# showlab/UniVTG

Hardware: NVIDIA H100
Metric: video-query pairs/sec (fwd+bwd) (higher is better)
Workload: dtype f16

## Files before the change

univtg_b200/csrc/backward.cu:

```cuda
#include <math.h>
#include <stdlib.h>

#include "backward.h"
#include "kernels.h"
#include "ptx.cuh"

namespace uv {

template <int EPT>
__global__ void __launch_bounds__(128) layernorm_bwd_kernel(const LnBwdArgs a) {
  pdl_prologue();
  const DropSpec drop = drop_resolve(a.drop);
  __shared__ float s_red[2][4];
  const int tid = threadIdx.x, warp = tid >> 5, lane = tid & 31;
  float acc_g[EPT], acc_b[EPT], acc_c[EPT];
#pragma unroll
  for (int i = 0; i < EPT; ++i) acc_g[i] = acc_b[i] = acc_c[i] = 0.f;
  const float inv_d = 1.0f / (float)a.d;

  for (int row = blockIdx.x; row < a.rows; row += gridDim.x) {
    const float mean = a.mean[row], rstd = a.rstd[row];
    const float* dout = a.dout + (size_t)row * a.ld_dout;
    const float* y = a.y + (size_t)row * a.ld_y;
    float xh[EPT], g[EPT];
// ... 101 lines not shown
    for (int i = 0; i < NV; ++i) {
      const int j = (tid + 128 * i) * 4;
      const bool in = j < a.d;
#define UV_LNB(c)                                          \
  xh[i].c = in ? (yv[i].c - mean) * rstd : 0.f;            \
  g[i].c = dj[i].c * gam[i].c;                             \
  acc_g[i].c += dj[i].c * xh[i].c;                         \
  acc_b[i].c += dj[i].c;                                   \
  s1 += g[i].c;                                            \
  s2 += g[i].c * xh[i].c;
      UV_LNB(x) UV_LNB(y) UV_LNB(z) UV_LNB(w)
#undef UV_LNB
    }
    s1 = warp_sum(s1);
    s2 = warp_sum(s2);
    __syncthreads();
    if (lane == 0) {
      s_red[0][warp] = s1;
      s_red[1][warp] = s2;
    }
    __syncthreads();
    const float c1 = (s_red[0][0] + s_red[0][1] + s_red[0][2] + s_red[0][3]) * inv_d;
    const float c2 = (s_red[1][0] + s_red[1][1] + s_red[1][2] + s_red[1][3]) * inv_d;
    float rs = 1.f;
    if (a.row_scale != nullptr) rs = a.row_scale[a.L > 0 ? row / a.L : 0];
#pragma unroll
    for (int i = 0; i < NV; ++i) {
      const int j = (tid + 128 * i) * 4;
      if (j < a.d) {
        float4 dy;
        dy.x = rstd * (g[i].x - c1 - xh[i].x * c2);
        dy.y = rstd * (g[i].y - c1 - xh[i].y * c2);
        dy.z = rstd * (g[i].z - c1 - xh[i].z * c2);
        dy.w = rstd * (g[i].w - c1 - xh[i].w * c2);
        if (a.relu_mask_y) {
          if (!(yv[i].x > 0.f)) dy.x = 0.f;
          if (!(yv[i].y > 0.f)) dy.y = 0.f;
          if (!(yv[i].z > 0.f)) dy.z = 0.f;
          if (!(yv[i].w > 0.f)) dy.w = 0.f;
        }
        if (a.dy32) *reinterpret_cast<float4*>(a.dy32 + (size_t)row * a.d + j) = dy;
        const float4 br = make_float4(dy.x * rs, dy.y * rs, dy.z * rs, dy.w * rs);
        acc_c[i].x += br.x, acc_c[i].y += br.y, acc_c[i].z += br.z, acc_c[i].w += br.w;
        if (a.dbr16)
          *reinterpret_cast<uint2*>(a.dbr16 + (size_t)row * a.ld16 + j) =
              make_uint2(cvt16x2(br.x, br.y, a.fmt16), cvt16x2(br.z, br.w, a.fmt16));
      }
    }
    if (a.dbr16)
      for (int j = a.d + tid; j < a.ld16; j += 128) a.dbr16[(size_t)row * a.ld16 + j] = 0;
  }
#pragma unroll
  for (int i = 0; i < NV; ++i) {
    const int j = (tid + 128 * i) * 4;
    if (j < a.d) {
      const float ps = a.pgrad_scale;
      if (a.dgamma) red_add_f32x4(a.dgamma + j, make_float4(acc_g[i].x * ps, acc_g[i].y * ps, acc_g[i].z * ps, acc_g[i].w * ps));
      if (a.dbeta) red_add_f32x4(a.dbeta + j, make_float4(acc_b[i].x * ps, acc_b[i].y * ps, acc_b[i].z * ps, acc_b[i].w * ps));
      if (a.colsum) red_add_f32x4(a.colsum + j, make_float4(acc_c[i].x * ps, acc_c[i].y * ps, acc_c[i].z * ps, acc_c[i].w * ps));
    }
  }
}

template <int NV>
__global__ void __launch_bounds__(256) layernorm_bwd_warp_kernel(const LnBwdArgs a) {
  pdl_prologue();
  const DropSpec drop = drop_resolve(a.drop);
  extern __shared__ float s_part[];
  const int tid = threadIdx.x, warp = tid >> 5, lane = tid & 31;
  constexpr int D = NV * 128;
  float4 acc_g[NV], acc_b[NV], acc_c[NV];
#pragma unroll
  for (int i = 0; i < NV; ++i) acc_g[i] = acc_b[i] = acc_c[i] = make_float4(0.f, 0.f, 0.f, 0.f);
  const float inv_d = 1.0f / (float)D;
  for (int row = blockIdx.x * 8 + warp; row < a.rows; row += gridDim.x * 8) {
    float4 g[NV], xh[NV];
#pragma unroll
    for (int i = 0; i < NV; ++i) {
      const int j = (i * 32 + lane) * 4;
      g[i] = __ldg(reinterpret_cast<const float4*>(a.dout + (size_t)row * a.ld_dout + j));
      xh[i] = __ldg(reinterpret_cast<const float4*>(a.y + (size_t)row * a.ld_y + j));
    }
    const float mean = a.mean[row], rstd = a.rstd[row];
    float rs = 1.f;
    if (a.row_scale != nullptr) rs = a.row_scale[a.L > 0 ? row / a.L : 0];
    float s1 = 0.f, s2 = 0.f;
    unsigned int relu = 0u;
#pragma unroll
    for (int i = 0; i < NV; ++i) {
      const int j = (i * 32 + lane) * 4;
      if (a.dout_mul) {
        const float4 m = __ldg(reinterpret_cast<const float4*>(a.dout_mul + (size_t)row * D + j));
        g[i].x *= m.x, g[i].y *= m.y, g[i].z *= m.z, g[i].w *= m.w;
      } else if (drop.on) {
        const float4 m = drop_mul4(drop, (unsigned int)row, (unsigned int)j);
        g[i].x *= m.x, g[i].y *= m.y, g[i].z *= m.z, g[i].w *= m.w;
      }
      const float4 gam = __ldg(reinterpret_cast<const float4*>(a.gamma + j));
#define UV_LNW(c, bit)                                  \
  if (xh[i].c > 0.f) relu |= 1u << (4 * i + bit);       \
  xh[i].c = (xh[i].c - mean) * rstd;                    \
  acc_g[i].c += g[i].c * xh[i].c;                       \
  acc_b[i].c += g[i].c;                                 \
  g[i].c *= gam.c;                                      \
  s1 += g[i].c;                                         \
  s2 += g[i].c * xh[i].c;
      UV_LNW(x, 0) UV_LNW(y, 1) UV_LNW(z, 2) UV_LNW(w, 3)
#undef UV_LNW
    }
    const float c1 = warp_sum(s1) * inv_d, c2 = warp_sum(s2) * inv_d;
#pragma unroll
    for (int i = 0; i < NV; ++i) {
      const int j = (i * 32 + lane) * 4;
      float4 dy;
      dy.x = rstd * (g[i].x - c1 - xh[i].x * c2);
      dy.y = rstd * (g[i].y - c1 - xh[i].y * c2);
      dy.z = rstd * (g[i].z - c1 - xh[i].z * c2);
      dy.w = rstd * (g[i].w - c1 - xh[i].w * c2);
      if (a.relu_mask_y) {
        if (!(relu & (1u << (4 * i + 0)))) dy.x = 0.f;
        if (!(relu & (1u << (4 * i + 1)))) dy.y = 0.f;
        if (!(relu & (1u << (4 * i + 2)))) dy.z = 0.f;
        if (!(relu & (1u << (4 * i + 3)))) dy.w = 0.f;
      }
      if (a.dy32) *reinterpret_cast<float4*>(a.dy32 + (size_t)row * D + j) = dy;
      const float4 br = make_float4(dy.x * rs, dy.y * rs, dy.z * rs, dy.w * rs);
      acc_c[i].x += br.x, acc_c[i].y += br.y, acc_c[i].z += br.z, acc_c[i].w += br.w;
      if (a.dbr16)
        *reinterpret_cast<uint2*>(a.dbr16 + (size_t)row * a.ld16 + j) = make_uint2(cvt16x2(br.x, br.y, a.fmt16), cvt16x2(br.z, br.w, a.fmt16));
    }
  }
  auto flush = [&](const float4 (&acc)[NV], float* dst) {
    if (dst == nullptr) return;
    __syncthreads();
#pragma unroll
    for (int i = 0; i < NV; ++i) *reinterpret_cast<float4*>(s_part + (size_t)warp * D + (i * 32 + lane) * 4) = acc[i];
    __syncthreads();
    for (int j = tid * 4; j < D; j += 256 * 4) {
      float4 t = make_float4(0.f, 0.f, 0.f, 0.f);
#pragma unroll
      for (int w = 0; w < 8; ++w) {
        const float4 v = *reinterpret_cast<const float4*>(s_part + (size_t)w * D + j);
        t.x += v.x, t.y += v.y, t.z += v.z, t.w += v.w;
      }
      const float ps = a.pgrad_scale;
      red_add_f32x4(dst + j, make_float4(t.x * ps, t.y * ps, t.z * ps, t.w * ps));
    }
  };
  flush(acc_g, a.dgamma);
  flush(acc_b, a.dbeta);
  flush(acc_c, a.colsum);
}

constexpr int kLnParamRows = 16;
__global__ void __launch_bounds__(256) layernorm_bwd_params_kernel(const LnBwdArgs a) {
  pdl_prologue();
  const DropSpec drop = drop_resolve(a.drop);
  const int jj = blockIdx.x * 256 + threadIdx.x;
  const bool in = jj < a.d;
  const int j = in ? jj : a.d - 1;
  const int r0 = blockIdx.y * kLnParamRows;
  const int r1 = min(a.rows, r0 + kLnParamRows);
  float ag = 0.f, ab = 0.f;
#pragma unroll
  for (int rr = 0; rr < kLnParamRows; ++rr) {
    const int r = r0 + rr;
    if (r >= r1) break;
    float dj = __ldg(a.dout + (size_t)r * a.ld_dout + j);
    if (a.dout_mul) dj *= __ldg(a.dout_mul + (size_t)r * a.d + j);
    else if (drop.on) {
      uint4 blk = make_uint4(0u, 0u, 0u, 0u);
      if ((threadIdx.x & 7) == 0) blk = drop_block(drop, (unsigned int)r, (unsigned int)(jj >> 3));
      const int src = (threadIdx.x & 31) & ~7;
      blk.x = __shfl_sync(0xffffffffu, blk.x, src);
      blk.y = __shfl_sync(0xffffffffu, blk.y, src);
      blk.z = __shfl_sync(0xffffffffu, blk.z, src);
      blk.w = __shfl_sync(0xffffffffu, blk.w, src);
      dj *= drop_pick(drop, blk, (unsigned int)(j & 7));
    }
    const float yv = a.y16 ? ld16(__ldg(a.y16 + (size_t)r * a.ld_y + j), a.y_fmt) : __ldg(a.y + (size_t)r * a.ld_y + j);
    const float xh = (yv - __ldg(a.mean + r)) * __ldg(a.rstd + r);
    ag += dj * xh;
    ab += dj;
  }
  if (in && a.dgamma) atomicAdd(a.dgamma + j, ag * a.pgrad_scale);
  if (in && a.dbeta) atomicAdd(a.dbeta + j, ab * a.pgrad_scale);
}

int launch_layernorm_bwd(const LnBwdArgs& a, cudaStream_t stream, int* kernel_used) {
  if (a.rows <= 0) return 0;
  if (a.dy32 == nullptr && a.dbr16 == nullptr) {
    if (kernel_used) *kernel_used = LNB_PARAMS;
    launch_k(layernorm_bwd_params_kernel, dim3(dim3((a.d + 255) / 256, (a.rows + kLnParamRows - 1) / kLnParamRows)), dim3(256), 0, stream, a);
    cudaError_t e = cudaGetLastError();
    if (e != cudaSuccess) set_error("layernorm_bwd launch failed: %s", cudaGetErrorString(e));
    return (int)e;
  }
  if (a.y16 != nullptr) {
    set_error("layernorm_bwd: a 16-bit LayerNorm input is only supported for the first projector layer (parameter gradients only)");
    return (int)cudaErrorInvalidValue;
  }
  static int max_blocks = 0;
  if (max_blocks == 0) {
    const char* e = getenv("UNIVTG_LNB_GRID");
    max_blocks = (e != nullptr && atoi(e) > 0) ? atoi(e) : 592;
  }
  const int grid = a.rows < max_blocks ? a.rows : max_blocks;
  const bool vec = a.d % 4 == 0 && a.ld_dout % 4 == 0 && a.ld_y % 4 == 0 && (!a.dbr16 || a.ld16 % 4 == 0) &&
                   (((uintptr_t)a.dout | (uintptr_t)a.y | (uintptr_t)a.gamma | (uintptr_t)a.dy32 | (uintptr_t)a.dout_mul) & 15) == 0 &&
                   (((uintptr_t)a.dgamma | (uintptr_t)a.dbeta | (uintptr_t)a.colsum) & 15) == 0 && ((uintptr_t)a.dbr16 & 7) == 0;
  static int use_warp = -1;
  if (use_warp < 0) {
    const char* e = getenv("UNIVTG_LNB_WARP");
    use_warp = (e != nullptr && e[0] == '0') ? 0 : 1;
  }
  const bool warp_ok = use_warp && vec && (a.d == 256 || a.d == 512 || a.d == 1024) && (!a.dbr16 || a.ld16 == a.d);
  if (warp_ok) {
    int dev = 0, sms = 132;
    cudaGetDevice(&dev);
    cudaDeviceGetAttribute(&sms, cudaDevAttrMultiProcessorCount, dev);
    int wgrid = (a.rows + 7) / 8;
    if (wgrid > sms) wgrid = sms;
    const size_t smem = (size_t)8 * a.d * sizeof(float);
    if (a.d == 1024) launch_k(layernorm_bwd_warp_kernel<8>, dim3(wgrid), dim3(256), smem, stream, a);
    else if (a.d == 512) launch_k(layernorm_bwd_warp_kernel<4>, dim3(wgrid), dim3(256), smem, stream, a);
    else launch_k(layernorm_bwd_warp_kernel<2>, dim3(wgrid), dim3(256), smem, stream, a);
    if (kernel_used) *kernel_used = a.d == 1024 ? LNB_WARP8 : (a.d == 512 ? LNB_WARP4 : LNB_WARP2);
  } else if (vec && a.d <= 512) {
    launch_k(layernorm_bwd_vec_kernel<1>, dim3(grid), dim3(128), 0, stream, a);
    if (kernel_used) *kernel_used = LNB_VEC1;
  } else if (vec && a.d <= 1024) {
    launch_k(layernorm_bwd_vec_kernel<2>, dim3(grid), dim3(128), 0, stream, a);
    if (kernel_used) *kernel_used = LNB_VEC2;
  } else if (a.d <= 128 * 8) {
    launch_k(layernorm_bwd_kernel<8>, dim3(grid), dim3(128), 0, stream, a);
    if (kernel_used) *kernel_used = LNB_ROW8;
  } else if (a.d <= 128 * 24) {
    launch_k(layernorm_bwd_kernel<24>, dim3(grid), dim3(128), 0, stream, a);
    if (kernel_used) *kernel_used = LNB_ROW24;
  } else {
    set_error("layernorm_bwd: d %d > 3072 not supported", a.d);
    return (int)cudaErrorInvalidValue;
  }
  cudaError_t e = cudaGetLastError();
  if (e != cudaSuccess) set_error("layernorm_bwd launch failed: %s", cudaGetErrorString(e));
  return (int)e;
}

__device__ __forceinline__ long long txt_row(const TxtRows& t, int r) {
  const int b = r / t.L, l = r - b * t.L;
  return l >= t.Lv ? (long long)b * (t.L - t.Lv) + (l - t.Lv) : -1;
}

template <bool TXT>
__global__ void __launch_bounds__(256) cvt16_colsum_kernel(const float* __restrict__ in32, int ld_in, uint16_t* __restrict__ out16,
                                                          int ld_out, int rows, int cols, int fmt, float* __restrict__ colsum, float cscale,
                                                          const TxtRows txt) {
  pdl_prologue();
  const int c = (blockIdx.x * 256 + threadIdx.x) * 4;
  if (c >= cols) return;
  const int r0 = blockIdx.y * 32;
  float4 s = make_float4(0.f, 0.f, 0.f, 0.f);
  for (int r = r0; r < min(rows, r0 + 32); ++r) {
    const float4 v = *reinterpret_cast<const float4*>(in32 + (size_t)r * ld_in + c);
    const uint2 h = make_uint2(cvt16x2(v.x, v.y, fmt), cvt16x2(v.z, v.w, fmt));
    *reinterpret_cast<uint2*>(out16 + (size_t)r * ld_out + c) = h;
    if constexpr (TXT) {
      const long long tr = txt_row(txt, r);
      if (tr >= 0 && c < txt.txt_cols) *reinterpret_cast<uint2*>(txt.txt16 + tr * txt.txt_cols + c) = h;
    }
    s.x += v.x;
    s.y += v.y;
    s.z += v.z;
    s.w += v.w;
  }
  if (colsum) {
    atomicAdd(colsum + c, s.x * cscale);
    atomicAdd(colsum + c + 1, s.y * cscale);
    atomicAdd(colsum + c + 2, s.z * cscale);
    atomicAdd(colsum + c + 3, s.w * cscale);
  }
}

__global__ void __launch_bounds__(256) tap_interleave_kernel(const float* __restrict__ src, float* __restrict__ dst, size_t nc) {
  pdl_prologue();
  for (size_t i = (size_t)blockIdx.x * 256 + threadIdx.x; i < nc; i += (size_t)gridDim.x * 256) {
    const float a = __ldg(src + i), b = __ldg(src + nc + i), c = __ldg(src + 2 * nc + i);
    float* o = dst + 3 * i;
    o[0] = a;
    o[1] = b;
    o[2] = c;
  }
}
int launch_tap_interleave(const float* src, float* dst, int N, int C, cudaStream_t stream) {
  const size_t nc = (size_t)N * C;
  size_t blocks = (nc + 255) / 256;
  if (blocks > 2368) blocks = 2368;
  launch_k(tap_interleave_kernel, dim3((unsigned)blocks), dim3(256), 0, stream, src, dst, nc);
  cudaError_t e = cudaGetLastError();
  if (e != cudaSuccess) set_error("tap_interleave launch failed: %s", cudaGetErrorString(e));
  return (int)e;
}

constexpr int kColsumRows = 16;
template <bool TXT>
__global__ void __launch_bounds__(128) colsum16_kernel(const uint16_t* __restrict__ in16, int ld, int rows, int cols, int fmt,
                                                      float* __restrict__ colsum, float scale, const TxtRows txt) {
  pdl_prologue();
  const int c = (blockIdx.x * 128 + threadIdx.x) * 8;
  if (c >= cols) return;
  const int r0 = blockIdx.y * kColsumRows;
  uint4 q[kColsumRows];
#pragma unroll
  for (int k = 0; k < kColsumRows; ++k)
    q[k] = (r0 + k < rows) ? __ldg(reinterpret_cast<const uint4*>(in16 + (size_t)(r0 + k) * ld + c)) : make_uint4(0u, 0u, 0u, 0u);
  if constexpr (TXT) {
    if (c < txt.txt_cols) {
#pragma unroll
      for (int k = 0; k < kColsumRows; ++k) {
        const long long tr = r0 + k < rows ? txt_row(txt, r0 + k) : -1;
        if (tr >= 0) *reinterpret_cast<uint4*>(txt.txt16 + tr * txt.txt_cols + c) = q[k];
      }
    }
  }
  float s[8] = {0.f, 0.f, 0.f, 0.f, 0.f, 0.f, 0.f, 0.f};
#pragma unroll
  for (int k = 0; k < kColsumRows; ++k) {
    const uint32_t w[4] = {q[k].x, q[k].y, q[k].z, q[k].w};
#pragma unroll
    for (int i = 0; i < 4; ++i) {
      s[2 * i] += ld16((uint16_t)(w[i] & 0xffff), fmt);
      s[2 * i + 1] += ld16((uint16_t)(w[i] >> 16), fmt);
    }
  }
  red_add_f32x4(colsum + c, make_float4(s[0] * scale, s[1] * scale, s[2] * scale, s[3] * scale));
  red_add_f32x4(colsum + c + 4, make_float4(s[4] * scale, s[5] * scale, s[6] * scale, s[7] * scale));
}

int launch_colsum16(const uint16_t* in16, int ld, int rows, int cols, int fmt, float* colsum, float scale, cudaStream_t stream,
                    TxtRows txt) {
  if (cols % 8 != 0 || ld % 8 != 0 || (reinterpret_cast<uintptr_t>(in16) & 15) != 0 || (reinterpret_cast<uintptr_t>(colsum) & 15) != 0 ||
      (txt.txt16 && (txt.txt_cols % 8 != 0 || (reinterpret_cast<uintptr_t>(txt.txt16) & 15) != 0))) {
    set_error("colsum16: columns / leading dimension must be multiples of 8 and the pointers 16-byte aligned");
    return (int)cudaErrorInvalidValue;
  }
  const dim3 grid((cols / 8 + 127) / 128, (rows + kColsumRows - 1) / kColsumRows);
// ... 34 lines not shown
      const int c0 = base + lane * 8;
      const bool in = c0 < d;
      const uint4 x = in ? __ldg(reinterpret_cast<const uint4*>(dO + (size_t)row * d + c0)) : make_uint4(0u, 0u, 0u, 0u);
      const uint4 y = in ? __ldg(reinterpret_cast<const uint4*>(O + (size_t)row * d + c0)) : make_uint4(0u, 0u, 0u, 0u);
      const uint32_t xw[4] = {x.x, x.y, x.z, x.w}, yw[4] = {y.x, y.y, y.z, y.w};
      float s = 0.f;
#pragma unroll
      for (int k = 0; k < 4; ++k)
        s += ld16((uint16_t)(xw[k] & 0xffff), fmt_do) * ld16((uint16_t)(yw[k] & 0xffff), fmt_o) +
             ld16((uint16_t)(xw[k] >> 16), fmt_do) * ld16((uint16_t)(yw[k] >> 16), fmt_o);
      for (int o = lph >> 1; o > 0; o >>= 1) s += __shfl_xor_sync(0xffffffffu, s, o);
      if (in && (lane & (lph - 1)) == 0) delta[((size_t)b * H + c0 / dh) * L + i] = s;
    }
    return;
  }
  for (int h = 0; h < H; ++h) {
    float s = 0.f;
    for (int c = lane; c < dh; c += 32) {
      const size_t idx = (size_t)row * d + h * dh + c;
      s += ld16(dO[idx], fmt_do) * ld16(O[idx], fmt_o);
    }
    s = warp_sum(s);
    if (lane == 0) delta[((size_t)b * H + h) * L + i] = s;
  }
}

int launch_attn_delta(const uint16_t* dO, int fmt_do, const uint16_t* O, int fmt_o, float* delta, int B, int L, int H, int dh,
                      cudaStream_t stream, int* vec_used) {
  const int rows = B * L;
  const int d = H * dh;
  const int vec = (dh % 8 == 0) && ((dh / 8) & (dh / 8 - 1)) == 0 && dh <= 256 && (d % 8 == 0) && (256 % dh == 0 || dh == 256) &&
                  ((reinterpret_cast<uintptr_t>(dO) | reinterpret_cast<uintptr_t>(O)) & 15) == 0;
  if (vec_used) *vec_used = vec;
  launch_k(attn_delta_kernel, dim3((rows * 32 + 255) / 256), dim3(256), 0, stream, dO, fmt_do, O, fmt_o, delta, B, L, H, dh, vec ? 1 : 0);
  cudaError_t e = cudaGetLastError();
  if (e != cudaSuccess) set_error("attn_delta launch failed: %s", cudaGetErrorString(e));
  return (int)e;
}

template <int DROP>
__global__ void __launch_bounds__(128) attention_bwd_simt_kernel(const AttnBwdArgs a) {
  pdl_prologue();
  const DropSpec drop = drop_resolve(a.drop);
  extern __shared__ float s_buf[];
  const int warp = threadIdx.x >> 5, lane = threadIdx.x & 31;
  const int gw = blockIdx.x * 4 + warp;
  if (gw >= a.B * a.H * a.L) return;
  const int i = gw % a.L;
  const int h = (gw / a.L) % a.H;
  const int b = gw / (a.L * a.H);
  float* p_s = s_buf + (size_t)warp * 2 * a.L;
  float* ds_s = p_s + a.L;
  const size_t ld = (size_t)3 * a.d;
  const uint16_t* qrow = a.qkv + ((size_t)b * a.L + i) * ld + h * a.dh;
  const uint16_t* dorow = a.dO + ((size_t)b * a.L + i) * a.d + h * a.dh;
  const float lse = a.lse[((size_t)b * a.H + h) * a.L + i];
  const float dlt = a.delta[((size_t)b * a.H + h) * a.L + i];
  for (int j = lane; j < a.L; j += 32) {
    float p = 0.f, ds = 0.f;
    if (a.key_mask[(size_t)b * a.L + j] != 0.f) {
      const uint16_t* krow = a.qkv + ((size_t)b * a.L + j) * ld + a.d + h * a.dh;
      const uint16_t* vrow = a.qkv + ((size_t)b * a.L + j) * ld + 2 * a.d + h * a.dh;
      float s = 0.f, dp = 0.f;
      for (int c = 0; c < a.dh; ++c) {
        s += ld16(qrow[c], a.fmt_act) * ld16(krow[c], a.fmt_act);
        dp += ld16(dorow[c], a.fmt_grad) * ld16(vrow[c], a.fmt_act);
      }
      p = expf(s * a.scale - lse);
      if constexpr (DROP != 0) {
        const float m = attn_drop_mul1(drop, (unsigned int)(b * a.H + h), (unsigned int)i, (unsigned int)j);
        ds = p * (m * dp - dlt) * a.scale;
        p *= m;
      } else {
        ds = p * (dp - dlt) * a.scale;
      }
    }
    p_s[j] = p;
    ds_s[j] = ds;
  }
  __syncwarp();
  for (int c = lane; c < a.dh; c += 32) {
    const float qc = ld16(qrow[c], a.fmt_act);
    const float doc = ld16(dorow[c], a.fmt_grad);
    float dq = 0.f;
    for (int j = 0; j < a.L; ++j) {
      const float ds = ds_s[j], p = p_s[j];
      if (p == 0.f && ds == 0.f) continue;
      const size_t kbase = ((size_t)b * a.L + j) * ld;
      dq += ds * ld16(a.qkv[kbase + a.d + h * a.dh + c], a.fmt_act);
      atomicAdd(a.dqkv32 + kbase + a.d + h * a.dh + c, ds * qc);
      atomicAdd(a.dqkv32 + kbase + 2 * a.d + h * a.dh + c, p * doc);
    }
    atomicAdd(a.dqkv32 + ((size_t)b * a.L + i) * ld + h * a.dh + c, dq);
  }
}

int launch_attention_bwd_simt(const AttnBwdArgs& a, cudaStream_t stream, int* kernel_used) {
  const int warps = a.B * a.H * a.L;
  const size_t smem = attention_bwd_simt_smem(a.L);
  auto kern = a.drop.on ? attention_bwd_simt_kernel<1> : attention_bwd_simt_kernel<0>;
  if (kernel_used) *kernel_used = 8 + (a.drop.on ? 1 : 0);
  if (smem > 48 * 1024) {
    cudaError_t e = cudaFuncSetAttribute(kern, cudaFuncAttributeMaxDynamicSharedMemorySize, (int)smem);
    if (e != cudaSuccess) {
      set_error("attention_bwd_simt smem %zu: %s", smem, cudaGetErrorString(e));
      return (int)e;
    }
  }
  launch_k(kern, dim3((warps + 3) / 4), dim3(128), smem, stream, a);
  cudaError_t e = cudaGetLastError();
  if (e != cudaSuccess) set_error("attention_bwd_simt launch failed: %s", cudaGetErrorString(e));
  return (int)e;
}

__global__ void __launch_bounds__(256) head_dz_kernel(const HeadFinalBwdArgs a) {
  pdl_prologue();
  const int idx = blockIdx.x * blockDim.x + threadIdx.x;
  const int rows = a.B * (a.Lv + 1) + 2;
  if (idx >= rows) return;
  float4 out = make_float4(0.f, 0.f, 0.f, 0.f);
  const int m = idx - 1;
  if (m >= 0 && m < a.B * (a.Lv + 1)) {
    const int b = m / (a.Lv + 1), l = m - b * (a.Lv + 1);
    if (l < a.Lv) {
      const size_t k = (size_t)b * a.Lv + l;
      const float pc = a.pred_logits[k];
      const float s0 = -a.pred_spans[2 * k];
      const float s1 = a.pred_spans[2 * k + 1];
      out.x = a.in_scale * a.g_logits[k] * pc * (1.f - pc);
      out.y = -a.in_scale * a.g_spans[2 * k] * s0 * (1.f - s0);
      out.z = a.in_scale * a.g_spans[2 * k + 1] * s1 * (1.f - s1);
    }
  }
  *reinterpret_cast<float4*>(a.dz + (size_t)idx * 4) = out;
}

__global__ void __launch_bounds__(256) head_dh_kernel(const HeadFinalBwdArgs a) {
  pdl_prologue();
  const int gw = (blockIdx.x * blockDim.x + threadIdx.x) >> 5;
  const int lane = threadIdx.x & 31;
  const int Mh = a.B * (a.Lv + 1);
  if (gw >= Mh) return;
  const size_t row = (size_t)gw + 1;
  const int l = gw % (a.Lv + 1);
  const bool sep = (l == a.Lv);
  float dzc[3], dz0[3], dz1[3];
#pragma unroll
  for (int t = 0; t < 3; ++t) {
    const float4 v = *reinterpret_cast<const float4*>(a.dz + (row + 1 - t) * 4);
    dzc[t] = v.x;
    dz0[t] = v.y;
    dz1[t] = v.z;
  }
  for (int c = lane * 2; c < a.d; c += 64) {
    float gc[2] = {0.f, 0.f}, gs[2] = {0.f, 0.f};
    if (!sep) {
#pragma unroll
      for (int t = 0; t < 3; ++t) {
#pragma unroll
        for (int e = 0; e < 2; ++e) {
          gc[e] += dzc[t] * a.w_cls[(size_t)t * a.d + c + e];
          gs[e] += dz0[t] * a.w_span[(size_t)t * a.d + c + e] + dz1[t] * a.w_span[(size_t)(3 + t) * a.d + c + e];
        }
      }
      const uint32_t hc = *reinterpret_cast<const uint32_t*>(a.h_cls + row * a.d + c);
      const uint32_t hs = *reinterpret_cast<const uint32_t*>(a.h_span + row * a.d + c);
      if (!pos16((uint16_t)(hc & 0xffff))) gc[0] = 0.f;
      if (!pos16((uint16_t)(hc >> 16))) gc[1] = 0.f;
      if (!pos16((uint16_t)(hs & 0xffff))) gs[0] = 0.f;
      if (!pos16((uint16_t)(hs >> 16))) gs[1] = 0.f;
    }
    *reinterpret_cast<uint32_t*>(a.dh_cls + row * a.d + c) = cvt16x2(gc[0], gc[1], a.fmt_grad);
    *reinterpret_cast<uint32_t*>(a.dh_span + row * a.d + c) = cvt16x2(gs[0], gs[1], a.fmt_grad);
  }
}

constexpr int kHeadDwRows = 32;
__device__ __forceinline__ void ld8(const uint16_t* p, int fmt, float (&v)[8]) {
  const uint4 q = *reinterpret_cast<const uint4*>(p);
  const uint32_t w[4] = {q.x, q.y, q.z, q.w};
#pragma unroll
  for (int i = 0; i < 4; ++i) {
    v[2 * i] = ld16((uint16_t)(w[i] & 0xffff), fmt);
    v[2 * i + 1] = ld16((uint16_t)(w[i] >> 16), fmt);
  }
}
__global__ void __launch_bounds__(128) head_dw_kernel(const HeadFinalBwdArgs a) {
  pdl_prologue();
  const int c = (blockIdx.x * 128 + threadIdx.x) * 8;
  const int Mh = a.B * (a.Lv + 1);
  const int m0 = blockIdx.y * kHeadDwRows;
  const int m1 = min(Mh, m0 + kHeadDwRows);
  if (c < a.d) {
    float wc[3][8], w0[3][8], w1[3][8], cs_c[8], cs_s[8];
#pragma unroll
    for (int j = 0; j < 8; ++j) {
      cs_c[j] = cs_s[j] = 0.f;
#pragma unroll
      for (int t = 0; t < 3; ++t) wc[t][j] = w0[t][j] = w1[t][j] = 0.f;
    }
    float pc[8], cc[8], nc[8], ps[8], cu[8], ns[8];
    ld8(a.h_cls + (size_t)m0 * a.d + c, a.fmt_act, pc);
    ld8(a.h_span + (size_t)m0 * a.d + c, a.fmt_act, ps);
    ld8(a.h_cls + (size_t)(m0 + 1) * a.d + c, a.fmt_act, cc);
    ld8(a.h_span + (size_t)(m0 + 1) * a.d + c, a.fmt_act, cu);
    for (int m = m0; m < m1; ++m) {
      const size_t row = (size_t)m + 1;
      ld8(a.h_cls + (row + 1) * a.d + c, a.fmt_act, nc);
      ld8(a.h_span + (row + 1) * a.d + c, a.fmt_act, ns);
      const float4 dz = *reinterpret_cast<const float4*>(a.dz + row * 4);
      if (a.cs_cls) {
        float gc[8], gs[8];
        ld8(a.dh_cls + row * a.d + c, a.fmt_grad, gc);
        ld8(a.dh_span + row * a.d + c, a.fmt_grad, gs);
#pragma unroll
        for (int j = 0; j < 8; ++j) {
          cs_c[j] += gc[j];
          cs_s[j] += gs[j];
        }
      }
      if (dz.x != 0.f || dz.y != 0.f || dz.z != 0.f) {
#pragma unroll
        for (int j = 0; j < 8; ++j) {
          wc[0][j] += dz.x * pc[j];
          wc[1][j] += dz.x * cc[j];
          wc[2][j] += dz.x * nc[j];
          w0[0][j] += dz.y * ps[j];
          w0[1][j] += dz.y * cu[j];
          w0[2][j] += dz.y * ns[j];
          w1[0][j] += dz.z * ps[j];
          w1[1][j] += dz.z * cu[j];
          w1[2][j] += dz.z * ns[j];
        }
      }
#pragma unroll
      for (int j = 0; j < 8; ++j) {
        pc[j] = cc[j];
        cc[j] = nc[j];
        ps[j] = cu[j];
        cu[j] = ns[j];
      }
    }
    const float gsc = a.pgrad_scale;
    float* dsts[3] = {a.gw_cls + (size_t)c * 3, a.gw_span + (size_t)c * 3, a.gw_span + ((size_t)a.d + c) * 3};
#pragma unroll
    for (int w = 0; w < 3; ++w) {
      float flat[24];
#pragma unroll
      for (int j = 0; j < 8; ++j)
#pragma unroll
        for (int t = 0; t < 3; ++t) flat[j * 3 + t] = (w == 0 ? wc[t][j] : (w == 1 ? w0[t][j] : w1[t][j])) * gsc;
#pragma unroll
      for (int q = 0; q < 6; ++q)
        red_add_f32x4(dsts[w] + 4 * q, make_float4(flat[4 * q], flat[4 * q + 1], flat[4 * q + 2], flat[4 * q + 3]));
    }
    if (a.cs_cls) {
      red_add_f32x4(a.cs_cls + c, make_float4(cs_c[0] * gsc, cs_c[1] * gsc, cs_c[2] * gsc, cs_c[3] * gsc));
      red_add_f32x4(a.cs_cls + c + 4, make_float4(cs_c[4] * gsc, cs_c[5] * gsc, cs_c[6] * gsc, cs_c[7] * gsc));
      red_add_f32x4(a.cs_span + c, make_float4(cs_s[0] * gsc, cs_s[1] * gsc, cs_s[2] * gsc, cs_s[3] * gsc));
      red_add_f32x4(a.cs_span + c + 4, make_float4(cs_s[4] * gsc, cs_s[5] * gsc, cs_s[6] * gsc, cs_s[7] * gsc));
    }
  }
  if (blockIdx.x == 0 && threadIdx.x == 0) {
    float bc = 0.f, b0 = 0.f, b1 = 0.f;
    for (int m = m0; m < m1; ++m) {
      const float4 dz = *reinterpret_cast<const float4*>(a.dz + ((size_t)m + 1) * 4);
      bc += dz.x;
      b0 += dz.y;
      b1 += dz.z;
    }
    atomicAdd(a.gb_cls, bc * a.pgrad_scale);
    atomicAdd(a.gb_span, b0 * a.pgrad_scale);
    atomicAdd(a.gb_span + 1, b1 * a.pgrad_scale);
  }
}

int launch_head_final_bwd(const HeadFinalBwdArgs& a, cudaStream_t stream) {
  const int Mh = a.B * (a.Lv + 1);
  launch_k(head_dz_kernel, dim3((Mh + 2 + 255) / 256), dim3(256), 0, stream, a);
  launch_k(head_dh_kernel, dim3((Mh * 32 + 255) / 256), dim3(256), 0, stream, a);
  launch_k(head_dw_kernel, dim3((a.d + 1023) / 1024, (Mh + kHeadDwRows - 1) / kHeadDwRows), dim3(128), 0, stream, a);
  cudaError_t e = cudaGetLastError();
  if (e != cudaSuccess) set_error("head_final_bwd launch failed: %s", cudaGetErrorString(e));
  return (int)e;
}

__global__ void __launch_bounds__(256) pool_bwd_kernel(const PoolBwdArgs a) {
  pdl_prologue();
  extern __shared__ float sm[];
  float* s_da = sm;
  __shared__ float s_dot;
  const int b = blockIdx.x;
  const int warp = threadIdx.x >> 5, lane = threadIdx.x & 31, nw = blockDim.x >> 5;
  const float* xt = a.x_txt + (size_t)b * a.Lt * a.d;
  const float* g = a.g_pooled + (size_t)b * a.d;
  const float* al = a.alpha + (size_t)b * a.Lt;
  for (int l = warp; l < a.Lt; l += nw) {
    float s = 0.f;
    for (int j = lane; j < a.d; j += 32) s += g[j] * xt[(size_t)l * a.d + j];
    s = warp_sum(s);
    if (lane == 0) s_da[l] = s;
  }
  __syncthreads();
  if (warp == 0) {
    float s = 0.f;
    for (int l = lane; l < a.Lt; l += 32) s += al[l] * s_da[l];
    s = warp_sum(s);
    if (lane == 0) s_dot = s;
  }
  __syncthreads();
  const float dot = s_dot;
  for (int l = threadIdx.x; l < a.Lt; l += blockDim.x) s_da[l] = al[l] * (s_da[l] - dot);
  __syncthreads();
  for (int j = threadIdx.x; j < a.d; j += blockDim.x) {
    const float gj = g[j], wj = a.w[j];
    float dw = 0.f;
    for (int l = 0; l < a.Lt; ++l) {
      const float dl = s_da[l];
      a.dx_txt[((size_t)b * a.Lt + l) * a.d + j] = (al[l] * gj + dl * wj) * a.out_scale;
      dw += dl * xt[(size_t)l * a.d + j];
    }
    atomicAdd(a.gw + j, dw);
  }
}

int launch_pool_bwd(const PoolBwdArgs& a, cudaStream_t stream) {
  launch_k(pool_bwd_kernel, dim3(a.B), dim3(256), (size_t)a.Lt * sizeof(float), stream, a);
  cudaError_t e = cudaGetLastError();
  if (e != cudaSuccess) set_error("pool_bwd launch failed: %s", cudaGetErrorString(e));
  return (int)e;
}

__global__ void __launch_bounds__(256) stream_gather_kernel(const float* __restrict__ dx, int L, int off, const float* __restrict__ extra,
                                                           float extra_scale, uint16_t* __restrict__ out16,
                                                           float* __restrict__ colsum, float cscale, int B, int Ls, int d, int fmt) {
  pdl_prologue();
  const int c = (blockIdx.x * 256 + threadIdx.x) * 4;
  if (c >= d) return;
  const int r0 = blockIdx.y * 32;
  const int rows = B * Ls;
  float4 s = make_float4(0.f, 0.f, 0.f, 0.f);
  for (int r = r0; r < min(rows, r0 + 32); ++r) {
    const int b = r / Ls, l = r - b * Ls;
    float4 v = *reinterpret_cast<const float4*>(dx + ((size_t)b * L + off + l) * d + c);
    if (extra) {
      const float4 e = *reinterpret_cast<const float4*>(extra + (size_t)r * d + c);
      v.x += e.x * extra_scale;
      v.y += e.y * extra_scale;
      v.z += e.z * extra_scale;
      v.w += e.w * extra_scale;
    }
    *reinterpret_cast<uint2*>(out16 + (size_t)r * d + c) = make_uint2(cvt16x2(v.x, v.y, fmt), cvt16x2(v.z, v.w, fmt));
    s.x += v.x;
    s.y += v.y;
    s.z += v.z;
    s.w += v.w;
  }
  if (colsum) {
    atomicAdd(colsum + c, s.x * cscale);
    atomicAdd(colsum + c + 1, s.y * cscale);
    atomicAdd(colsum + c + 2, s.z * cscale);
    atomicAdd(colsum + c + 3, s.w * cscale);
  }
}

int launch_stream_gather(const float* dx_stream, int L, int off, const float* extra, float extra_scale, uint16_t* out16,
                         float* colsum, float colsum_scale, int B, int Ls, int d, int fmt, cudaStream_t stream) {
  dim3 grid((d / 4 + 255) / 256, (B * Ls + 31) / 32);
  launch_k(stream_gather_kernel, dim3(grid), dim3(256), 0, stream, dx_stream, L, off, extra, extra_scale, out16, colsum, colsum_scale, B, Ls, d, fmt);
  cudaError_t e = cudaGetLastError();
  if (e != cudaSuccess) set_error("stream_gather launch failed: %s", cudaGetErrorString(e));
  return (int)e;
}


template <int EPT>
__global__ void __launch_bounds__(128) txt_pos_bwd_kernel(const TxtPosBwdArgs a) {
  pdl_prologue();
  const DropSpec drop = drop_resolve(a.drop);
  __shared__ float s_red[2][2][4];
  const int l = blockIdx.x;
  const int tid = threadIdx.x, warp = tid >> 5, lane = tid & 31;
  const float* P = a.table + (size_t)l * a.d;
  float acc_p[EPT], acc_g[EPT], acc_b[EPT], pv[EPT], gam[EPT];
#pragma unroll
  for (int i = 0; i < EPT; ++i) {
    const int j = tid + 128 * i;
    acc_p[i] = acc_g[i] = acc_b[i] = 0.f;
    pv[i] = j < a.d ? P[j] : 0.f;
    gam[i] = j < a.d ? a.gamma[j] : 0.f;
  }
  for (int b = 0; b < a.B; ++b) {
    const size_t r = (size_t)b * a.Lt + l;
    const float mean = a.mean[r], rstd = a.rstd[r];
    float g[EPT], xh[EPT];
    float s1 = 0.f, s2 = 0.f;
#pragma unroll
    for (int i = 0; i < EPT; ++i) {
      const int j = tid + 128 * i;
      g[i] = xh[i] = 0.f;
      if (j < a.d) {
        float go = a.dpos[r * a.d + j];
        if (a.mul32) go *= a.mul32[r * a.d + j];
        else if (drop.on) go *= drop_mul1(drop, (unsigned int)r, (unsigned int)j);
        xh[i] = (a.xt[r * a.d + j] + pv[i] - mean) * rstd;
        acc_g[i] += go * xh[i];
        acc_b[i] += go;
        g[i] = go * gam[i];
        s1 += g[i];
        s2 += g[i] * xh[i];
      }
    }
    s1 = warp_sum(s1);
    s2 = warp_sum(s2);
    if (lane == 0) {
      s_red[b & 1][0][warp] = s1;
      s_red[b & 1][1][warp] = s2;
    }
    __syncthreads();
    const float m1 = (s_red[b & 1][0][0] + s_red[b & 1][0][1] + s_red[b & 1][0][2] + s_red[b & 1][0][3]) / (float)a.d;
    const float m2 = (s_red[b & 1][1][0] + s_red[b & 1][1][1] + s_red[b & 1][1][2] + s_red[b & 1][1][3]) / (float)a.d;
    float* dxr = a.dx + ((size_t)b * a.L + a.Lv + l) * a.d;
#pragma unroll
    for (int i = 0; i < EPT; ++i) {
      const int j = tid + 128 * i;
      if (j < a.d) {
        const float du = rstd * (g[i] - m1 - xh[i] * m2);
        acc_p[i] += du;
        dxr[j] += du;
      }
    }
  }
#pragma unroll
  for (int i = 0; i < EPT; ++i) {
    const int j = tid + 128 * i;
    if (j < a.d) {
      a.dtable[(size_t)l * a.d + j] = acc_p[i] * a.pgrad_scale;
      atomicAdd(a.dgamma + j, acc_g[i] * a.pgrad_scale);
      atomicAdd(a.dbeta + j, acc_b[i] * a.pgrad_scale);
    }
  }
}

int launch_txt_pos_bwd(const TxtPosBwdArgs& a, cudaStream_t stream) {
  if (a.d > 128 * 8) {
    set_error("txt_pos_bwd: hidden_dim %d > 1024 not supported", a.d);
    return (int)cudaErrorInvalidValue;
  }
  launch_k(txt_pos_bwd_kernel<8>, dim3(a.Lt), dim3(128), 0, stream, a);
  cudaError_t e = cudaGetLastError();
  if (e != cudaSuccess) set_error("txt_pos_bwd launch failed: %s", cudaGetErrorString(e));
  return (int)e;
}

}
```

univtg_b200/csrc/loss.cu:

```cuda
#include <math.h>

#include "kernels.h"
#include "loss.h"
#include "ptx.cuh"

namespace uv {

__global__ void __launch_bounds__(256) loss_cos_kernel(const LossArgs a) {
  pdl_prologue();
  const int gw = (blockIdx.x * blockDim.x + threadIdx.x) >> 5;
  const int lane = threadIdx.x & 31;
  const int n_in = a.B * a.Lv;
  if (gw >= n_in + a.B * a.B) return;
  int bv, lv, bt;
  if (gw < n_in) {
    bv = gw / a.Lv;
    lv = gw - bv * a.Lv;
    bt = bv;
  } else {
    const int k = gw - n_in;
    bv = k / a.B;
    bt = k - bv * a.B;
    lv = (int)a.pos_idx[bv];
  }
// ... 212 lines not shown
  v = warp_max(v);
  __syncthreads();
  if ((threadIdx.x & 31) == 0) s_red[threadIdx.x >> 5] = v;
  __syncthreads();
  float t = -INFINITY;
  const int nw = blockDim.x >> 5;
  for (int i = 0; i < nw; ++i) t = fmaxf(t, s_red[i]);
  return t;
}

__global__ void __launch_bounds__(1024) qfvs_loss_kernel(const QfvsLossArgs a) {
  pdl_prologue();
  __shared__ float s_red[32];
  __shared__ int s_cnt[32];
  const int tid = threadIdx.x, nt = blockDim.x, lane = tid & 31, warp = tid >> 5, nw = nt >> 5;
  const int n = a.B * a.Lv;
  const float inv_tau = 1.0f / a.temperature;
  int ranked = 0;
  float c_t = 0.f, c_pos = 0.f, c_bce = 0.f, c_zpos = 0.f, mx = -INFINITY, se = 0.f;
  for (int base = 0; base < n; base += nt) {
    const int i = base + tid;
    const bool keep = i < n && a.mask_gt[i] != 0;
    const unsigned bal = __ballot_sync(0xffffffffu, keep);
    if (lane == 0) s_cnt[warp] = __popc(bal);
    __syncthreads();
    int before = 0, total = 0;
    for (int w = 0; w < nw; ++w) {
      const int c = s_cnt[w];
      before += w < warp ? c : 0;
      total += c;
    }
    __syncthreads();
    if (i < n) {
      float t = 0.f;
      if (keep) {
        t = a.sal[ranked + before + __popc(bal & ((1u << lane) - 1u))];
        const float p = a.pred_logits[i];
        const float lp = fmaxf(logf(p), -100.f), l1p = fmaxf(logf(1.f - p), -100.f);
        c_t += t;
        c_bce += -(t * lp + (1.f - t) * l1p);
        const float z = (a.cos_in[i] + logf(a.vmask[i] + 1e-45f)) * inv_tau;
        if (t > 0.f) {
          c_pos += 1.f;
          c_zpos += z;
        }
        if (z > mx) {
          se = se * expf(mx - z) + 1.f;
          mx = z;
        } else {
          se += expf(z - mx);
        }
      }
      a.g_logits_f[i] = t;
      a.g_cos_in[i] = keep ? 1.f : 0.f;
    }
    ranked += total;
  }
  const float sum_t = block_sum(c_t, s_red);
  const float n_pos = block_sum(c_pos, s_red);
  const float bce = block_sum(c_bce, s_red);
  const float zpos = block_sum(c_zpos, s_red);
  const float zmax = block_max(mx, s_red);
  const float lse = zmax + logf(block_sum(mx == -INFINITY ? 0.f : se * expf(mx - zmax), s_red));
  const bool on = sum_t != 0.f;
  const bool sal_on = on && a.has_pos != 0;
  for (int i = tid; i < n; i += nt) {
    const float t = a.g_logits_f[i];
    const bool keep = a.g_cos_in[i] != 0.f;
    float gf = 0.f, gc = 0.f;
    if (keep && on) {
      const float p = a.pred_logits[i];
      gf = (p - t) / fmaxf(p * (1.f - p), 1e-12f) / sum_t;
    }
    if (keep && sal_on) {
      const float z = (a.cos_in[i] + logf(a.vmask[i] + 1e-45f)) * inv_tau;
      gc = (expf(z - lse) - (t > 0.f ? 1.f / n_pos : 0.f)) * inv_tau;
    }
    a.g_logits_f[i] = gf;
    a.g_cos_in[i] = gc;
    a.g_spans_b[2 * i] = 0.f;
    a.g_spans_b[2 * i + 1] = 0.f;
    a.g_spans_g[2 * i] = 0.f;
    a.g_spans_g[2 * i + 1] = 0.f;
  }
  if (tid == 0) {
    a.losses[0] = 0.f;
    a.losses[1] = 0.f;
    a.losses[2] = on ? bce / sum_t : 0.f;
    a.losses[3] = 0.f;
    a.losses[4] = sal_on ? lse - zpos / n_pos : 0.f;
  }
}

int launch_qfvs_loss_forward(const QfvsLossArgs& q, cudaStream_t stream) {
  LossArgs c = {};
  c.xv = q.xv;
  c.xt = q.xt;
  c.B = q.B;
  c.Lv = q.Lv;
  c.d = q.d;
  c.cos_in = q.cos_in;
  c.vnorm = q.vnorm;
  c.tnorm = q.tnorm;
  launch_k(loss_cos_kernel, dim3(q.B * q.Lv), dim3(32), 0, stream, c);
  launch_k(qfvs_loss_kernel, dim3(1), dim3(1024), 0, stream, q);
  cudaError_t e = cudaGetLastError();
  if (e != cudaSuccess) set_error("qfvs loss forward launch failed: %s", cudaGetErrorString(e));
  return (int)e;
}

__global__ void __launch_bounds__(256) loss_bwd_small_kernel(const LossBwdArgs a) {
  pdl_prologue();
  const int i = blockIdx.x * blockDim.x + threadIdx.x;
  const int n = a.B * a.Lv;
  if (i >= n) return;
  const float wb = a.w[0], wg = a.w[1], wf = a.w[2];
  a.d_logits[i] = wf * a.g_logits_f[i];
  a.d_spans[2 * i] = wb * a.g_spans_b[2 * i] + wg * a.g_spans_g[2 * i];
  a.d_spans[2 * i + 1] = wb * a.g_spans_b[2 * i + 1] + wg * a.g_spans_g[2 * i + 1];
}

__global__ void __launch_bounds__(256) loss_bwd_vid_kernel(const LossBwdArgs a) {
  pdl_prologue();
  const int gw = (blockIdx.x * blockDim.x + threadIdx.x) >> 5;
  const int lane = threadIdx.x & 31;
  if (gw >= a.B * a.Lv) return;
  const int b = gw / a.Lv, l = gw - b * a.Lv;
  const float w_inter = a.w[3], w_intra = a.w[4];
  const float un = a.vnorm[gw];
  const float gi = w_intra * a.g_cos_in[gw];
  const float ci = a.cos_in[gw];
  const bool is_pos = a.pos_idx != nullptr && (int)a.pos_idx[b] == l;
  const float* u = a.xv + (size_t)gw * a.d;
  float* out = a.d_xv + (size_t)gw * a.d;
  extern __shared__ float s_c1[];
  float* c1w = s_c1 + (size_t)(threadIdx.x >> 5) * a.B;
  const float s1 = gi / (un * a.tnorm[b]);
  float s2 = gi * ci / (un * un);
  if (is_pos) {
    float s2p = 0.f;
    for (int k = lane; k < a.B; k += 32) {
      const float gx = w_inter * a.g_sim[b * a.B + k];
      c1w[k] = gx / (un * a.tnorm[k]);
      s2p += gx * a.sim[b * a.B + k] / (un * un);
    }
    s2 += warp_sum(s2p);
    __syncwarp();
  }
  for (int j = lane * 4; j < a.d; j += 128) {
    const float4 x = *reinterpret_cast<const float4*>(u + j);
    const float4 t = *reinterpret_cast<const float4*>(a.xt + (size_t)b * a.d + j);
    float4 o = make_float4(s1 * t.x, s1 * t.y, s1 * t.z, s1 * t.w);
    if (is_pos) {
#pragma unroll 4
      for (int k = 0; k < a.B; ++k) {
        const float4 tk = *reinterpret_cast<const float4*>(a.xt + (size_t)k * a.d + j);
        const float c1 = c1w[k];
        o.x += c1 * tk.x;
        o.y += c1 * tk.y;
        o.z += c1 * tk.z;
        o.w += c1 * tk.w;
      }
    }
    o.x -= s2 * x.x;
    o.y -= s2 * x.y;
    o.z -= s2 * x.z;
    o.w -= s2 * x.w;
    *reinterpret_cast<float4*>(out + j) = o;
  }
}

__global__ void __launch_bounds__(128) loss_bwd_txt_kernel(const LossBwdArgs a) {
  pdl_prologue();
  extern __shared__ float s_coef[];
  int* s_row = reinterpret_cast<int*>(s_coef + a.Lv + a.B);
  __shared__ float s_red[4];
  const int b = blockIdx.x, tid = threadIdx.x;
  const float w_inter = a.w[3], w_intra = a.w[4];
  const float tn = a.tnorm[b];
  float part = 0.f;
  for (int l = tid; l < a.Lv; l += 128) {
    const int i = b * a.Lv + l;
    const float g = w_intra * a.g_cos_in[i];
    s_coef[l] = g / (a.vnorm[i] * tn);
    part += g * a.cos_in[i];
  }
  const int nk = a.pos_idx != nullptr ? a.B : 0;
  for (int k = tid; k < nk; k += 128) {
    const float g = w_inter * a.g_sim[k * a.B + b];
    const int i = k * a.Lv + (int)a.pos_idx[k];
    s_coef[a.Lv + k] = g / (a.vnorm[i] * tn);
    s_row[k] = i;
    part += g * a.sim[k * a.B + b];
  }
  part = warp_sum(part);
  if ((tid & 31) == 0) s_red[tid >> 5] = part;
  __syncthreads();
  const float c2 = (s_red[0] + s_red[1] + s_red[2] + s_red[3]) / (tn * tn);
  for (int j = blockIdx.y * 128 + tid; j < a.d; j += gridDim.y * 128) {
    float o = -c2 * a.xt[(size_t)b * a.d + j];
    const float* xv = a.xv + (size_t)b * a.Lv * a.d + j;
#pragma unroll 8
    for (int l = 0; l < a.Lv; ++l) o += s_coef[l] * xv[(size_t)l * a.d];
#pragma unroll 4
    for (int k = 0; k < nk; ++k) o += s_coef[a.Lv + k] * a.xv[(size_t)s_row[k] * a.d + j];
    a.d_xt[(size_t)b * a.d + j] = o;
  }
}

int launch_loss_backward(const LossBwdArgs& a, cudaStream_t stream) {
  const int n = a.B * a.Lv;
  launch_k(loss_bwd_small_kernel, dim3((n + 255) / 256), dim3(256), 0, stream, a);
  if (a.pos_idx == nullptr) {
    cudaMemsetAsync(a.d_xv, 0, (size_t)n * a.d * sizeof(float), stream);
    cudaMemsetAsync(a.d_xt, 0, (size_t)a.B * a.d * sizeof(float), stream);
    cudaError_t e0 = cudaGetLastError();
    if (e0 != cudaSuccess) set_error("loss backward launch failed: %s", cudaGetErrorString(e0));
    return (int)e0;
  }
  launch_k(loss_bwd_vid_kernel, dim3((n * 32 + 255) / 256), dim3(256), (size_t)8 * a.B * sizeof(float), stream, a);
  launch_k(loss_bwd_txt_kernel, dim3(a.B, (a.d + 127) / 128), dim3(128), (size_t)(a.Lv + 2 * a.B) * sizeof(float), stream, a);
  cudaError_t e = cudaGetLastError();
  if (e != cudaSuccess) set_error("loss backward launch failed: %s", cudaGetErrorString(e));
  return (int)e;
}

int launch_qfvs_loss_backward(const LossBwdArgs& a, cudaStream_t stream) {
  const int n = a.B * a.Lv;
  launch_k(loss_bwd_small_kernel, dim3((n + 255) / 256), dim3(256), 0, stream, a);
  launch_k(loss_bwd_vid_kernel, dim3((n * 32 + 255) / 256), dim3(256), (size_t)8 * a.B * sizeof(float), stream, a);
  launch_k(loss_bwd_txt_kernel, dim3(a.B, (a.d + 127) / 128), dim3(128), (size_t)(a.Lv + 2 * a.B) * sizeof(float), stream, a);
  cudaError_t e = cudaGetLastError();
  if (e != cudaSuccess) set_error("qfvs loss backward launch failed: %s", cudaGetErrorString(e));
  return (int)e;
}

}
```

Before: 6818.

## Restructure LN param-grad, stream gather and pool backward kernels for more parallelism and ILP

The LayerNorm parameter-gradient kernel now has each thread handle 8 columns with vectorized loads. It batches rows for memory-level parallelism, reduces across warps in shared memory, and picks rows-per-slice so the grid fills the SMs. The stream gather kernel also reduces in shared memory before issuing atomics and preloads several rows per thread. Pool backward is split across a second grid dimension over columns, and two loops get higher unroll pragmas. The aim is fewer global atomics and more parallelism in small backward kernels, at the cost of more registers and shared memory.

```diff
diff --git a/univtg_b200/csrc/backward.cu b/univtg_b200/csrc/backward.cu
--- a/univtg_b200/csrc/backward.cu
+++ b/univtg_b200/csrc/backward.cu
@@ -277,46 +277,91 @@
   flush(acc_c, a.colsum);
 }
 
-constexpr int kLnParamRows = 16;
-__global__ void __launch_bounds__(256) layernorm_bwd_params_kernel(const LnBwdArgs a) {
+constexpr int kLnParamBatch = 4;
+__global__ void __launch_bounds__(256) layernorm_bwd_params_kernel(const LnBwdArgs a, int rows_per_slice) {
   pdl_prologue();
   const DropSpec drop = drop_resolve(a.drop);
-  const int jj = blockIdx.x * 256 + threadIdx.x;
-  const bool in = jj < a.d;
-  const int j = in ? jj : a.d - 1;
-  const int r0 = blockIdx.y * kLnParamRows;
-  const int r1 = min(a.rows, r0 + kLnParamRows);
-  float ag = 0.f, ab = 0.f;
-#pragma unroll
-  for (int rr = 0; rr < kLnParamRows; ++rr) {
-    const int r = r0 + rr;
-    if (r >= r1) break;
-    float dj = __ldg(a.dout + (size_t)r * a.ld_dout + j);
-    if (a.dout_mul) dj *= __ldg(a.dout_mul + (size_t)r * a.d + j);
-    else if (drop.on) {
-      uint4 blk = make_uint4(0u, 0u, 0u, 0u);
-      if ((threadIdx.x & 7) == 0) blk = drop_block(drop, (unsigned int)r, (unsigned int)(jj >> 3));
-      const int src = (threadIdx.x & 31) & ~7;
-      blk.x = __shfl_sync(0xffffffffu, blk.x, src);
-      blk.y = __shfl_sync(0xffffffffu, blk.y, src);
-      blk.z = __shfl_sync(0xffffffffu, blk.z, src);
-      blk.w = __shfl_sync(0xffffffffu, blk.w, src);
-      dj *= drop_pick(drop, blk, (unsigned int)(j & 7));
-    }
-    const float yv = a.y16 ? ld16(__ldg(a.y16 + (size_t)r * a.ld_y + j), a.y_fmt) : __ldg(a.y + (size_t)r * a.ld_y + j);
-    const float xh = (yv - __ldg(a.mean + r)) * __ldg(a.rstd + r);
-    ag += dj * xh;
-    ab += dj;
-  }
-  if (in && a.dgamma) atomicAdd(a.dgamma + j, ag * a.pgrad_scale);
-  if (in && a.dbeta) atomicAdd(a.dbeta + j, ab * a.pgrad_scale);
+  __shared__ float s_acc[2][8][256];
+  const int tx = threadIdx.x & 31, ty = threadIdx.x >> 5;
+  const int j0 = (blockIdx.x * 32 + tx) * 8;
+  const int nc = max(0, min(8, a.d - j0));
+  const bool dvec = nc == 8 && (a.ld_dout & 3) == 0 && ((uintptr_t)a.dout & 15) == 0 && !a.dout_mul;
+  const bool yvec = nc == 8 && !a.y16 && (a.ld_y & 1) == 0 && ((uintptr_t)a.y & 7) == 0;
+  const int r0 = (blockIdx.y * 8 + ty) * rows_per_slice;
+  const int r1 = nc > 0 ? min(a.rows, r0 + rows_per_slice) : r0;
+  float ag[8], ab[8];
+#pragma unroll
+  for (int k = 0; k < 8; ++k) ag[k] = ab[k] = 0.f;
+  for (int rb = r0; rb < r1; rb += kLnParamBatch) {
+    float g[kLnParamBatch][8], y[kLnParamBatch][8];
+#pragma unroll
+    for (int q = 0; q < kLnParamBatch; ++q) {
+      const int r = min(rb + q, r1 - 1);
+      const float* dr = a.dout + (size_t)r * a.ld_dout + j0;
+      if (dvec) {
+        const float4 u = __ldg(reinterpret_cast<const float4*>(dr)), v = __ldg(reinterpret_cast<const float4*>(dr + 4));
+        g[q][0] = u.x, g[q][1] = u.y, g[q][2] = u.z, g[q][3] = u.w, g[q][4] = v.x, g[q][5] = v.y, g[q][6] = v.z, g[q][7] = v.w;
+      } else {
+#pragma unroll
+        for (int k = 0; k < 8; ++k) g[q][k] = k < nc ? __ldg(dr + k) * (a.dout_mul ? __ldg(a.dout_mul + (size_t)r * a.d + j0 + k) : 1.f) : 0.f;
+      }
+      if (yvec) {
+        const float* yr = a.y + (size_t)r * a.ld_y + j0;
+#pragma unroll
+        for (int k = 0; k < 4; ++k) {
+          const float2 t = __ldg(reinterpret_cast<const float2*>(yr + 2 * k));
+          y[q][2 * k] = t.x, y[q][2 * k + 1] = t.y;
+        }
+      } else {
+#pragma unroll
+        for (int k = 0; k < 8; ++k) {
+          const size_t o = (size_t)r * a.ld_y + j0 + k;
+          y[q][k] = k < nc ? (a.y16 ? ld16(__ldg(a.y16 + o), a.y_fmt) : __ldg(a.y + o)) : 0.f;
+        }
+      }
+    }
+#pragma unroll
+    for (int q = 0; q < kLnParamBatch; ++q) {
+      const int r = rb + q;
+      if (r >= r1) break;
+      float m8[8] = {1.f, 1.f, 1.f, 1.f, 1.f, 1.f, 1.f, 1.f};
+      if (!a.dout_mul && drop.on) drop_mul8(drop, (unsigned int)r, (unsigned int)(j0 >> 3), m8);
+      const float mean = __ldg(a.mean + r), rstd = __ldg(a.rstd + r);
+#pragma unroll
+      for (int k = 0; k < 8; ++k) {
+        const float dj = g[q][k] * m8[k];
+        ag[k] += dj * ((y[q][k] - mean) * rstd);
+        ab[k] += dj;
+      }
+    }
+  }
+#pragma unroll
+  for (int k = 0; k < 8; ++k) {
+    s_acc[0][ty][tx * 8 + k] = ag[k];
+    s_acc[1][ty][tx * 8 + k] = ab[k];
+  }
+  __syncthreads();
+  const int c = threadIdx.x, j = blockIdx.x * 256 + c;
+  if (j < a.d) {
+    float tg = 0.f, tb = 0.f;
+#pragma unroll
+    for (int w = 0; w < 8; ++w) {
+      tg += s_acc[0][w][c];
+      tb += s_acc[1][w][c];
+    }
+    if (a.dgamma) atomicAdd(a.dgamma + j, tg * a.pgrad_scale);
+    if (a.dbeta) atomicAdd(a.dbeta + j, tb * a.pgrad_scale);
+  }
 }
 
 int launch_layernorm_bwd(const LnBwdArgs& a, cudaStream_t stream, int* kernel_used) {
   if (a.rows <= 0) return 0;
   if (a.dy32 == nullptr && a.dbr16 == nullptr) {
     if (kernel_used) *kernel_used = LNB_PARAMS;
-    launch_k(layernorm_bwd_params_kernel, dim3(dim3((a.d + 255) / 256, (a.rows + kLnParamRows - 1) / kLnParamRows)), dim3(256), 0, stream, a);
+    const int gx = (a.d + 255) / 256;
+    int rps = 16;
+    while (rps > kLnParamBatch && (long long)gx * ((a.rows + 8 * rps - 1) / (8 * rps)) < 2 * 132) rps -= kLnParamBatch;
+    launch_k(layernorm_bwd_params_kernel, dim3(gx, (a.rows + 8 * rps - 1) / (8 * rps)), dim3(256), 0, stream, a, rps);
     cudaError_t e = cudaGetLastError();
     if (e != cudaSuccess) set_error("layernorm_bwd launch failed: %s", cudaGetErrorString(e));
     return (int)e;
@@ -657,6 +702,7 @@
     dz0[t] = v.y;
     dz1[t] = v.z;
   }
+#pragma unroll 4
   for (int c = lane * 2; c < a.d; c += 64) {
     float gc[2] = {0.f, 0.f}, gs[2] = {0.f, 0.f};
     if (!sep) {
@@ -817,7 +863,7 @@
   const float dot = s_dot;
   for (int l = threadIdx.x; l < a.Lt; l += blockDim.x) s_da[l] = al[l] * (s_da[l] - dot);
   __syncthreads();
-  for (int j = threadIdx.x; j < a.d; j += blockDim.x) {
+  for (int j = blockIdx.y * blockDim.x + threadIdx.x; j < a.d; j += gridDim.y * blockDim.x) {
     const float gj = g[j], wj = a.w[j];
     float dw = 0.f;
     for (int l = 0; l < a.Lt; ++l) {
@@ -830,38 +876,59 @@
 }
 
 int launch_pool_bwd(const PoolBwdArgs& a, cudaStream_t stream) {
-  launch_k(pool_bwd_kernel, dim3(a.B), dim3(256), (size_t)a.Lt * sizeof(float), stream, a);
+  launch_k(pool_bwd_kernel, dim3(a.B, (a.d + 255) / 256), dim3(256), (size_t)a.Lt * sizeof(float), stream, a);
   cudaError_t e = cudaGetLastError();
   if (e != cudaSuccess) set_error("pool_bwd launch failed: %s", cudaGetErrorString(e));
   return (int)e;
 }
 
+constexpr int kGatherRows = 8;
 __global__ void __launch_bounds__(256) stream_gather_kernel(const float* __restrict__ dx, int L, int off, const float* __restrict__ extra,
                                                            float extra_scale, uint16_t* __restrict__ out16,
                                                            float* __restrict__ colsum, float cscale, int B, int Ls, int d, int fmt) {
   pdl_prologue();
-  const int c = (blockIdx.x * 256 + threadIdx.x) * 4;
-  if (c >= d) return;
-  const int r0 = blockIdx.y * 32;
+  __shared__ float4 s_sum[4][64];
+  const int tx = threadIdx.x & 63, ty = threadIdx.x >> 6;
+  const int c = (blockIdx.x * 64 + tx) * 4;
+  const int r0 = (blockIdx.y * 4 + ty) * kGatherRows;
   const int rows = B * Ls;
   float4 s = make_float4(0.f, 0.f, 0.f, 0.f);
-  for (int r = r0; r < min(rows, r0 + 32); ++r) {
-    const int b = r / Ls, l = r - b * Ls;
-    float4 v = *reinterpret_cast<const float4*>(dx + ((size_t)b * L + off + l) * d + c);
-    if (extra) {
-      const float4 e = *reinterpret_cast<const float4*>(extra + (size_t)r * d + c);
-      v.x += e.x * extra_scale;
-      v.y += e.y * extra_scale;
-      v.z += e.z * extra_scale;
-      v.w += e.w * extra_scale;
-    }
-    *reinterpret_cast<uint2*>(out16 + (size_t)r * d + c) = make_uint2(cvt16x2(v.x, v.y, fmt), cvt16x2(v.z, v.w, fmt));
-    s.x += v.x;
-    s.y += v.y;
-    s.z += v.z;
-    s.w += v.w;
-  }
-  if (colsum) {
+  if (c < d && r0 < rows) {
+    float4 v[kGatherRows];
+#pragma unroll
+    for (int k = 0; k < kGatherRows; ++k) {
+      const int r = min(r0 + k, rows - 1), b = r / Ls, l = r - b * Ls;
+      v[k] = *reinterpret_cast<const float4*>(dx + ((size_t)b * L + off + l) * d + c);
+      if (extra) {
+        const float4 e = *reinterpret_cast<const float4*>(extra + (size_t)r * d + c);
+        v[k].x += e.x * extra_scale;
+        v[k].y += e.y * extra_scale;
+        v[k].z += e.z * extra_scale;
+        v[k].w += e.w * extra_scale;
+      }
+    }
+#pragma unroll
+    for (int k = 0; k < kGatherRows; ++k) {
+      const int r = r0 + k;
+      if (r >= rows) break;
+      *reinterpret_cast<uint2*>(out16 + (size_t)r * d + c) = make_uint2(cvt16x2(v[k].x, v[k].y, fmt), cvt16x2(v[k].z, v[k].w, fmt));
+      s.x += v[k].x;
+      s.y += v[k].y;
+      s.z += v[k].z;
+      s.w += v[k].w;
+    }
+  }
+  if (colsum == nullptr) return;
+  s_sum[ty][tx] = s;
+  __syncthreads();
+  if (ty == 0 && c < d) {
+    for (int w = 1; w < 4; ++w) {
+      const float4 t = s_sum[w][tx];
+      s.x += t.x;
+      s.y += t.y;
+      s.z += t.z;
+      s.w += t.w;
+    }
     atomicAdd(colsum + c, s.x * cscale);
     atomicAdd(colsum + c + 1, s.y * cscale);
     atomicAdd(colsum + c + 2, s.z * cscale);
@@ -871,7 +938,7 @@
 
 int launch_stream_gather(const float* dx_stream, int L, int off, const float* extra, float extra_scale, uint16_t* out16,
                          float* colsum, float colsum_scale, int B, int Ls, int d, int fmt, cudaStream_t stream) {
-  dim3 grid((d / 4 + 255) / 256, (B * Ls + 31) / 32);
+  dim3 grid((d / 4 + 63) / 64, (B * Ls + 4 * kGatherRows - 1) / (4 * kGatherRows));
   launch_k(stream_gather_kernel, dim3(grid), dim3(256), 0, stream, dx_stream, L, off, extra, extra_scale, out16, colsum, colsum_scale, B, Ls, d, fmt);
   cudaError_t e = cudaGetLastError();
   if (e != cudaSuccess) set_error("stream_gather launch failed: %s", cudaGetErrorString(e));
diff --git a/univtg_b200/csrc/loss.cu b/univtg_b200/csrc/loss.cu
--- a/univtg_b200/csrc/loss.cu
+++ b/univtg_b200/csrc/loss.cu
@@ -388,7 +388,7 @@
     const float4 t = *reinterpret_cast<const float4*>(a.xt + (size_t)b * a.d + j);
     float4 o = make_float4(s1 * t.x, s1 * t.y, s1 * t.z, s1 * t.w);
     if (is_pos) {
-#pragma unroll 4
+#pragma unroll 16
       for (int k = 0; k < a.B; ++k) {
         const float4 tk = *reinterpret_cast<const float4*>(a.xt + (size_t)k * a.d + j);
         const float c1 = c1w[k];
```

After: 6972 (median of 6 runs). 1.02x the previous value.
